# A-SHOJAEI/preference-guided-image-captioning-alignment

Hardware: NVIDIA B200
Metric: dpo_pair_tokens_per_s (higher is better)
Workload: dtype bf16

## Files before the change

### include/pgica.h

```cpp
#ifndef PGICA_H_
#define PGICA_H_

#include <stddef.h>
#include <stdint.h>

#ifdef __cplusplus
extern "C" {
#endif

#define PGICA_ABI_VERSION 1

#define PGICA_OK 0
#define PGICA_ERR_INVALID_ARGUMENT (-1)
#define PGICA_ERR_CUDA (-2)
#define PGICA_ERR_UNSUPPORTED_DEVICE (-3)
#define PGICA_ERR_WORKSPACE_TOO_SMALL (-4)

#define PGICA_MASK_NONE 0
#define PGICA_MASK_I64 1
#define PGICA_MASK_F32 2
#define PGICA_MASK_U8 3
#define PGICA_MASK_I32 4

int pgica_abi_version(void);
// ... 47 lines not shown
int pgica_lmhead_logprob_fwd(const void* hidden, const void* weight, const int64_t* labels, const void* mask,
                             int mask_kind, int64_t nseq, int64_t seqlen, int64_t d, int64_t vocab,
                             int length_normalize, float* seq_logp, float* lse, float* ztgt, int32_t* row_label,
                             float* row_weight, float* nll_sum, void* workspace, size_t workspace_bytes,
                             void* stream);
int pgica_lmhead_logprob_bwd(const void* hidden, const void* weight, const int32_t* row_label,
                             const float* row_weight, const float* lse, const float* grad_seq, int64_t nseq,
                             int64_t seqlen, int64_t d, int64_t vocab, int length_normalize, void* dhidden,
                             int dhidden_is_bf16, void* dweight, int dweight_is_bf16, void* workspace,
                             size_t workspace_bytes, void* stream);
int pgica_lmhead_logprob_bwd_progress(const void* hidden, const void* weight, const int32_t* row_label,
                                      const float* row_weight, const float* lse, const float* grad_seq, int64_t nseq,
                                      int64_t seqlen, int64_t d, int64_t vocab, int length_normalize, void* dhidden,
                                      int dhidden_is_bf16, void* dweight, uint32_t* progress, int64_t rows_per_segment,
                                      int32_t* increments_per_256_rows_host, void* workspace, size_t workspace_bytes,
                                      void* stream);

int pgica_compact_rows(const float* row_weight, int64_t rows, int32_t* index, int32_t* count, void* stream);
int pgica_gather_rows_bf16(const void* src, int src_is_bf16, const int32_t* index, int64_t n, int64_t d,
                           void* dst_bf16, const int32_t* label_in, int32_t* label_out, void* stream);
int pgica_gather_u32(const void* src, const int32_t* index, int64_t n, void* dst, void* stream);
int pgica_scatter_u32(const void* src, const int32_t* index, int64_t n, void* dst, int64_t dst_n, void* stream);
int pgica_scatter_rows(const void* src, int src_is_bf16, const int32_t* index, int64_t n, int64_t d, void* dst,
                       int dst_is_bf16, int64_t dst_rows, void* stream);
int pgica_lmhead_rows_workspace_bytes(int64_t rows, int64_t d, int64_t vocab, size_t* bytes_host);
int pgica_lmhead_rows_bwd(const void* hidden, const void* weight, const int32_t* row_label, const float* lse,
                          const float* ncoef, int64_t rows, int64_t d, int64_t vocab, void* dhidden,
                          int dhidden_is_bf16, void* dweight, int dweight_is_bf16, void* workspace,
                          size_t workspace_bytes, void* stream);

int pgica_dpo_loss_fwd(const float* pc, const float* pr, const float* rc, const float* rr, int64_t n,
                       int64_t n_global, float beta, float label_smoothing, float* loss, float* metrics, float* dpc,
                       void* stream);

int pgica_ntxent_workspace_bytes(int64_t rows_a, int64_t rows_b, int64_t dim, size_t* bytes_host);
int pgica_ntxent_fwd(const void* a, const void* b, int64_t rows_a, int64_t rows_b, int64_t dim, float inv_tau,
                     int64_t diag_offset, float* lse_row, float* diag, float* lse_col_part, void* workspace,
                     size_t workspace_bytes, void* stream);
int pgica_ntxent_fwd_bounded(const void* a, const void* b, int64_t rows_a, int64_t rows_b, int64_t dim, float inv_tau,
                             int64_t diag_offset, float* lse_row, float* diag, float* lse_col_part, void* workspace,
                             size_t workspace_bytes, void* stream);
int pgica_ntxent_bwd(const void* a, const void* b, int64_t rows_a, int64_t rows_b, int64_t dim, float inv_tau,
                     int64_t diag_offset, const float* lse_row, const float* lse_col, const float* grad_loss,
                     float grad_mult, void* da, int da_is_bf16, void* db, int db_is_bf16, void* workspace,
                     size_t workspace_bytes, void* stream);
int pgica_ntxent_bwd_bounded(const void* a, const void* b, int64_t rows_a, int64_t rows_b, int64_t dim, float inv_tau,
                             int64_t diag_offset, const float* lse_row, const float* lse_col, const float* grad_loss,
                             float grad_mult, void* da, int da_is_bf16, void* db, int db_is_bf16, void* workspace,
                             size_t workspace_bytes, void* stream);
int pgica_ntxent_loss(const float* lse_row, const float* diag, const float* lse_col_owned, int64_t n,
                      float inv_denom, float* loss, void* stream);
int pgica_lse_combine(const float* parts, int64_t nparts, int64_t n, float* out, void* stream);
int pgica_ntxent_coef(const float* grad, float mult, int64_t n, int64_t tgt_offset, int64_t tgt_limit, float* coef,
                      int32_t* tgt, void* stream);

int pgica_rownorm_fwd(const void* x, int x_is_bf16, int64_t rows, int64_t dim, float eps, void* y_bf16,
                      float* inv_norm, void* left3_bf16, void* right3_bf16, void* stream);
int pgica_rownorm_bwd(const void* x, int x_is_bf16, const float* inv_norm, const void* g, int g_is_bf16, int64_t rows,
                      int64_t dim, int64_t g_pitch, int64_t g_second, float* dx, void* stream);
int pgica_cast_f32_to_bf16(const float* x, int64_t n, void* y_bf16, void* stream);
int pgica_split3_bf16(const float* x, int64_t rows, int64_t dim, void* left3_bf16, void* right3_bf16, void* stream);

int pgica_sum_into_f32(float* dst, const void* const* srcs_host, int n_src, int64_t n, int max_ctas, void* stream);

int pgica_prep_rows(const int64_t* labels, const void* mask, int mask_kind, int64_t nseq, int64_t seqlen,
                    int64_t vocab, int32_t* row_label, float* row_weight, void* stream);
// ... 48 lines not shown
```

### preference_guided_image_captioning_alignment_b200/csrc/gemm_lse.cu

```cuda
#include "common.h"
#include "ptx.cuh"

namespace pgica {

namespace {

constexpr int kBlockM = 128;
constexpr int kBlockN = 256;
constexpr int kBlockK = 64;
constexpr int kUmmaK = 16;
constexpr int kStages = 7;
constexpr int kAccStages = 2;
constexpr uint32_t kABytes = kBlockM * kBlockK * 2;
constexpr uint32_t kBBytes = (kBlockN / 2) * kBlockK * 2;
constexpr int kMaxEpiGroups = 2;
constexpr int epi_groups(bool cols) { return cols ? 2 : 1; }
constexpr int block_threads(bool cols) { return 128 + 128 * epi_groups(cols); }
constexpr int kEpilogueWarp0 = 4;
constexpr float kLn2 = 0.6931471805599453f;

struct GemmLseParams {
  int rows, cols, k;
  int num_m_blocks, num_m_pairs, num_n_tiles, rows_pad;
  int num_parts;
// ... 233 lines not shown
        run_m = m_new;
        if ((rel >> 5) == ch && rel >= 0) {
          const int jj = rel & 31;
          float z = 0.f;
#pragma unroll
          for (int j = 0; j < 32; ++j)
            if (j == jj) z = v[j];
          run_t = z * p.scale;
        }
      }
      tc_fence_before_sync();
      mbar_arrive_cluster(&tempty_bar[acc], 0);
      if (++acc == kAccStages) {
        acc = 0;
        acc_phase ^= 1;
      }
      if (m_blk < p.num_m_blocks) {
        const size_t o = (static_cast<size_t>(n_tile) * kEpiGroups + wg) * p.rows_pad + m_blk * kBlockM + row_in_blk;
        p.part_max[o] = run_m;
        p.part_sum[o] = run_s;
        p.part_tgt[o] = run_t;
      }
    }
  }

  tc_fence_before_sync();
  __syncthreads();
  cluster_sync_all();
  if (warp == 2)
    asm volatile("tcgen05.dealloc.cta_group::2.sync.aligned.b32 %0, %1;" ::"r"(tmem_base), "r"(kAccStages * kBlockN)
                 : "memory");
}

constexpr int kMergeRows = 32, kMergeGroups = 8;
__global__ void __launch_bounds__(kMergeRows* kMergeGroups)
lse_merge_kernel(const GemmLseParams p, float* __restrict__ lse, float* __restrict__ tgt) {
  __shared__ float s_m[kMergeGroups][kMergeRows], s_s[kMergeGroups][kMergeRows], s_t[kMergeGroups][kMergeRows];
  const int r = threadIdx.x % kMergeRows, g = threadIdx.x / kMergeRows;
  const int row = blockIdx.x * kMergeRows + r;
  float m = -INFINITY, sum = 0.f, t = -INFINITY;
  if (row < p.rows) {
    for (int s = g; s < p.num_parts; s += kMergeGroups) {
      const size_t o = static_cast<size_t>(s) * p.rows_pad + row;
      const float pm = p.part_max[o], ps = p.part_sum[o];
      if (pm == -INFINITY && ps == 0.f) continue;
      const float mn = fmaxf(m, pm);
      sum = sum * exp2f(m - mn) + ps * exp2f(pm - mn);
      m = mn;
      t = fmaxf(t, p.part_tgt[o]);
    }
  }
  s_m[g][r] = m;
  s_s[g][r] = sum;
  s_t[g][r] = t;
  __syncthreads();
  if (g == 0 && row < p.rows) {
    float M = -INFINITY;
#pragma unroll
    for (int i = 0; i < kMergeGroups; ++i) M = fmaxf(M, s_m[i][r]);
    float S = 0.f, T = -INFINITY;
    bool bad = false;
#pragma unroll
    for (int i = 0; i < kMergeGroups; ++i) {
      const float mi = s_m[i][r], si = s_s[i][r];
      bad |= (si != si) || (mi != mi);
      if (mi > -INFINITY) S += si * exp2f(mi - M);
      T = fmaxf(T, s_t[i][r]);
    }
    float out = (M + log2f(S)) * kLn2;
    if (bad) out = NAN;
    lse[row] = out;
    if (tgt) tgt[row] = (T == -INFINITY) ? 0.f : T;
  }
}

__global__ void __launch_bounds__(512) col_merge_kernel(const GemmLseParams p, int groups, float* __restrict__ lse_col) {
  __shared__ float sm_m[16][33], sm_s[16][33];
  const int tx = threadIdx.x & 31, ty = threadIdx.x >> 5;
  const int j = blockIdx.x * 32 + tx;
  const size_t shift_pitch = static_cast<size_t>(p.num_n_tiles) * 8;
  const int slot = blockIdx.x;
  float M = -INFINITY, S = 0.f;
  if (j < p.cols) {
#pragma unroll 4
    for (int g = ty; g < groups; g += 16) {
      const float sh = p.col_shift[g * shift_pitch + slot];
      const float v = p.col_sum[static_cast<size_t>(g) * p.cols_pad + j];
      if (sh > -INFINITY) {
        if (sh > M) {
          S = S * exp2f(M - sh) + v;
          M = sh;
        } else {
          S += v * exp2f(sh - M);
        }
      }
    }
  }
  sm_m[ty][tx] = M;
  sm_s[ty][tx] = S;
  __syncthreads();
  if (ty == 0 && j < p.cols) {
    float Mx = -INFINITY;
#pragma unroll
    for (int t = 0; t < 16; ++t) Mx = fmaxf(Mx, sm_m[t][tx]);
    float Sx = 0.f;
#pragma unroll
// ... 13 lines not shown
  p->k = (int)k;
  p->num_m_blocks = (int)ceil_div(rows, kBlockM);
  p->num_m_pairs = (p->num_m_blocks + 1) / 2;
  p->num_n_tiles = (int)ceil_div(cols, kBlockN);
  p->rows_pad = p->num_m_blocks * kBlockM;
  const int64_t total = (int64_t)p->num_m_pairs * p->num_n_tiles;
  PGICA_REQUIRE(total < (1ll << 30), "gemm_lse: too many tiles");
  const int pairs = device_sm_count() / 2;
  *grid = 2 * (int)(total < pairs ? total : pairs);
  *ws_bytes = 3 * align_up((size_t)p->num_n_tiles * kMaxEpiGroups * p->rows_pad * sizeof(float), 256);
  return PGICA_OK;
}

size_t col_stats_bytes(const GemmLseParams& p, size_t* sum_bytes) {
  const size_t groups = static_cast<size_t>(p.rows_pad) / 32;
  const size_t cols_pad = align_up((size_t)p.cols, 32);
  *sum_bytes = align_up(groups * cols_pad * sizeof(float), 256);
  return *sum_bytes + align_up(groups * (size_t)p.num_n_tiles * 8 * sizeof(float), 256);
}

}
}

extern "C" {

int pgica_gemm_lse_workspace_bytes(int64_t rows, int64_t cols, int64_t k, size_t* bytes_host) {
  pgica::GemmLseParams p{};
  int grid = 0;
  return pgica::plan(rows, cols, k, &p, &grid, bytes_host);
}

static int gemm_lse_impl(const void* a, const void* b, int64_t rows, int64_t cols, int64_t k, float scale,
                         const int32_t* labels, int64_t diag_offset, float* lse, float* tgt, float* z_out,
                         void* workspace, size_t workspace_bytes, void* stream, float* lse_col = nullptr) {
  using namespace pgica;
  int rc = pgica_device_check();
  if (rc != PGICA_OK) return rc;
  GemmLseParams p{};
  int grid = 0;
  size_t need = 0;
  rc = plan(rows, cols, k, &p, &grid, &need);
  if (rc != PGICA_OK) return rc;
  PGICA_REQUIRE(a && b && lse, "gemm_lse: null operand");
  PGICA_REQUIRE(scale > 0.f && scale == scale, "gemm_lse: scale must be positive (got %g)", (double)scale);
  size_t col_sum_bytes = 0;
  const size_t col_bytes = lse_col ? col_stats_bytes(p, &col_sum_bytes) : 0;
  if (workspace_bytes < need + col_bytes || !workspace) {
    set_error("gemm_lse: workspace too small (%zu < %zu)", workspace_bytes, need + col_bytes);
    return PGICA_ERR_WORKSPACE_TOO_SMALL;
  }
  if (lse_col) {
    p.col_sum = reinterpret_cast<float*>(static_cast<uint8_t*>(workspace) + need);
    p.col_shift = reinterpret_cast<float*>(static_cast<uint8_t*>(workspace) + need + col_sum_bytes);
    p.cols_pad = (int)align_up((size_t)cols, 32);
  }
  const size_t seg = need / 3;
  p.part_max = reinterpret_cast<float*>(workspace);
  p.part_sum = reinterpret_cast<float*>(static_cast<uint8_t*>(workspace) + seg);
  p.part_tgt = reinterpret_cast<float*>(static_cast<uint8_t*>(workspace) + 2 * seg);
  p.num_parts = p.num_n_tiles * epi_groups(lse_col != nullptr);
  p.scale = scale;
  p.labels = labels;
  p.diag_offset = (int)diag_offset;
  p.z_out = z_out;

  CUtensorMap tm_a, tm_b;
  rc = make_tmap_bf16(&tm_a, a, rows, k, k, kBlockM);
  if (rc != PGICA_OK) return rc;
  rc = make_tmap_bf16(&tm_b, b, cols, k, k, kBlockN / 2);
  if (rc != PGICA_OK) return rc;

  cudaStream_t st = static_cast<cudaStream_t>(stream);
  auto kern = lse_col ? gemm_lse_kernel<true> : gemm_lse_kernel<false>;
  PGICA_CUDA_OK(cudaFuncSetAttribute(kern, cudaFuncAttributeMaxDynamicSharedMemorySize, (int)kSmemBytes));
  cudaLaunchConfig_t cfg{};
  cfg.gridDim = dim3((unsigned)grid);
  cfg.blockDim = dim3(lse_col ? block_threads(true) : block_threads(false));
  cfg.dynamicSmemBytes = kSmemBytes;
  cfg.stream = st;
  cudaLaunchAttribute attr[1];
  attr[0].id = cudaLaunchAttributeClusterDimension;
  attr[0].val.clusterDim.x = 2;
  attr[0].val.clusterDim.y = 1;
  attr[0].val.clusterDim.z = 1;
  cfg.attrs = attr;
  cfg.numAttrs = 1;
  PGICA_CUDA_OK(cudaLaunchKernelEx(&cfg, kern, tm_a, tm_b, p));
  count_launches(1);
  lse_merge_kernel<<<(unsigned)ceil_div(rows, kMergeRows), kMergeRows * kMergeGroups, 0, st>>>(p, lse, tgt);
  PGICA_CUDA_OK(cudaGetLastError());
  count_launches(1);
  if (lse_col) {
    col_merge_kernel<<<(unsigned)ceil_div(cols, 32), 512, 0, st>>>(p, p.rows_pad / 32, lse_col);
    PGICA_CUDA_OK(cudaGetLastError());
    count_launches(1);
  }
  return PGICA_OK;
}

int pgica_gemm_lse_rowcol_workspace_bytes(int64_t rows, int64_t cols, int64_t k, size_t* bytes_host) {
  pgica::GemmLseParams p{};
  int grid = 0;
  size_t need = 0;
  int rc = pgica::plan(rows, cols, k, &p, &grid, &need);
  if (rc != PGICA_OK) return rc;
  PGICA_REQUIRE(bytes_host, "workspace query: null result pointer");
  size_t sum_bytes = 0;
  *bytes_host = need + pgica::col_stats_bytes(p, &sum_bytes);
  return PGICA_OK;
}

int pgica_gemm_lse_rowcol(const void* a, const void* b, int64_t rows, int64_t cols, int64_t k, float scale,
                          const int32_t* labels, int64_t diag_offset, float* lse_row, float* tgt, float* lse_col,
                          void* workspace, size_t workspace_bytes, void* stream) {
  PGICA_REQUIRE(lse_col, "gemm_lse_rowcol: null column output");
  return gemm_lse_impl(a, b, rows, cols, k, scale, labels, diag_offset, lse_row, tgt, nullptr, workspace,
                       workspace_bytes, stream, lse_col);
}

int pgica_gemm_lse(const void* a, const void* b, int64_t rows, int64_t cols, int64_t k, float scale,
                   const int32_t* labels, int64_t diag_offset, float* lse, float* tgt, void* workspace,
                   size_t workspace_bytes, void* stream) {
  return gemm_lse_impl(a, b, rows, cols, k, scale, labels, diag_offset, lse, tgt, nullptr, workspace,
                       workspace_bytes, stream);
}

int pgica_similarity(const void* a, const void* b, int64_t rows, int64_t cols, int64_t k, float scale, float* sim,
                     float* lse, void* workspace, size_t workspace_bytes, void* stream) {
  PGICA_REQUIRE(sim && lse, "similarity: null output");
  return gemm_lse_impl(a, b, rows, cols, k, scale, nullptr, 0, lse, nullptr, sim, workspace, workspace_bytes, stream);
}

}
```

### preference_guided_image_captioning_alignment_b200/csrc/heads.cu

```cuda
#include "common.h"
#include "sgg_tile.cuh"

namespace pgica {
size_t sggx_workspace_bytes();
bool sggf_supported(int64_t mx, int64_t my, int64_t k);
bool sggf_single_chunk(int64_t mx, int64_t my, int64_t k);
size_t sggf_workspace_bytes();
int sggf_dispatch(const void* x, const void* y, int64_t mx, int64_t my, int64_t k, const SoftmaxGradStats& stats,
                  void* out_x, int out_x_is_bf16, void* out_y, int out_y_is_bf16, void* workspace,
                  size_t workspace_bytes, cudaStream_t st, uint32_t* progress, int64_t rows_per_segment,
                  bool shared_exponential);

namespace {
size_t backward_workspace_bytes(int64_t mx, int64_t my, int64_t k) {
  const size_t one = sggx_workspace_bytes();
  return sggf_supported(mx, my, k) && sggf_workspace_bytes() > one ? sggf_workspace_bytes() : one;
}

int backward(const void* x, const void* y, int64_t mx, int64_t my, int64_t k, float scale, const SoftmaxGradStats& st,
             void* out_x, int out_x_is_bf16, void* out_y, int out_y_is_bf16, void* ws, size_t ws_bytes, void* stream,
             bool shared_exponential) {
  if (out_x && out_y && sggf_supported(mx, my, k) && ws && ws_bytes >= sggf_workspace_bytes() &&
      (!out_y_is_bf16 || sggf_single_chunk(mx, my, k))) {
    if (shared_exponential)
      return sggf_dispatch(x, y, mx, my, k, st, out_x, out_x_is_bf16, out_y, out_y_is_bf16, ws, ws_bytes,
                           static_cast<cudaStream_t>(stream), nullptr, 0, true);
    return pgica_softmax_grad_gemm_dual(x, y, mx, my, k, scale, st.r_lse, st.r_coef, st.r_tgt, st.c_lse, st.c_coef,
                                        st.c_tgt, out_x, out_x_is_bf16, out_y, out_y_is_bf16, ws, ws_bytes, stream);
  }
  int rc;
  if (out_x) {
    rc = pgica_softmax_grad_gemm(x, y, mx, my, k, scale, st.r_lse, st.r_coef, st.r_tgt, st.c_lse, st.c_coef, st.c_tgt,
                                 out_x, out_x_is_bf16, ws, ws_bytes, stream);
    if (rc != PGICA_OK) return rc;
  }
  if (out_y) {
    const SoftmaxGradStats t = st.transposed();
    rc = pgica_softmax_grad_gemm(y, x, my, mx, k, scale, t.r_lse, t.r_coef, t.r_tgt, t.c_lse, t.c_coef, t.c_tgt, out_y,
                                 out_y_is_bf16, ws, ws_bytes, stream);
    if (rc != PGICA_OK) return rc;
  }
  return PGICA_OK;
}
}
}

using namespace pgica;

extern "C" {


int pgica_lmhead_logprob_workspace_bytes(int64_t nseq, int64_t seqlen, int64_t d, int64_t vocab, size_t* bytes_host) {
  PGICA_REQUIRE(bytes_host, "workspace query: null result pointer");
  size_t g = 0;
  int rc = pgica_gemm_lse_workspace_bytes(nseq * seqlen, vocab, d, &g);
  if (rc != PGICA_OK) return rc;
  const size_t bwd =
      align_up((size_t)(nseq * seqlen) * sizeof(float), 256) + backward_workspace_bytes(nseq * seqlen, vocab, d);
  *bytes_host = g > bwd ? g : bwd;
  return PGICA_OK;
}

int pgica_lmhead_logprob_fwd(const void* hidden, const void* weight, const int64_t* labels, const void* mask,
                             int mask_kind, int64_t nseq, int64_t seqlen, int64_t d, int64_t vocab,
                             int length_normalize, float* seq_logp, float* lse, float* ztgt, int32_t* row_label,
                             float* row_weight, float* nll_sum, void* workspace, size_t workspace_bytes,
                             void* stream) {
  PGICA_REQUIRE(hidden && weight && labels && seq_logp && lse && ztgt && row_label && row_weight,
                "lmhead_logprob_fwd: null pointer");
  int rc = pgica_prep_rows(labels, mask, mask_kind, nseq, seqlen, vocab, row_label, row_weight, stream);
  if (rc != PGICA_OK) return rc;
  rc = pgica_gemm_lse(hidden, weight, nseq * seqlen, vocab, d, 1.0f, row_label, 0, lse, ztgt, workspace,
                      workspace_bytes, stream);
  if (rc != PGICA_OK) return rc;
  return pgica_seq_reduce(lse, ztgt, row_weight, nseq, seqlen, length_normalize, seq_logp, nll_sum, stream);
}

int pgica_lmhead_rows_workspace_bytes(int64_t rows, int64_t d, int64_t vocab, size_t* bytes_host) {
  return pgica_lmhead_logprob_workspace_bytes(rows, 1, d, vocab, bytes_host);
}

int pgica_lmhead_rows_bwd(const void* hidden, const void* weight, const int32_t* row_label, const float* lse,
                          const float* ncoef, int64_t rows, int64_t d, int64_t vocab, void* dhidden,
                          int dhidden_is_bf16, void* dweight, int dweight_is_bf16, void* workspace,
                          size_t workspace_bytes, void* stream) {
  PGICA_REQUIRE(hidden && weight && row_label && lse && ncoef, "lmhead_rows_bwd: null pointer");
  PGICA_REQUIRE(dhidden || dweight, "lmhead_rows_bwd: nothing to compute");
  return backward(hidden, weight, rows, vocab, d, 1.0f, {kLog2e, lse, ncoef, row_label, nullptr, nullptr, nullptr},
                  dhidden, dhidden_is_bf16, dweight, dweight_is_bf16, workspace, workspace_bytes, stream, false);
}

int pgica_lmhead_logprob_bwd(const void* hidden, const void* weight, const int32_t* row_label,
                             const float* row_weight, const float* lse, const float* grad_seq, int64_t nseq,
                             int64_t seqlen, int64_t d, int64_t vocab, int length_normalize, void* dhidden,
                             int dhidden_is_bf16, void* dweight, int dweight_is_bf16, void* workspace,
                             size_t workspace_bytes, void* stream) {
  PGICA_REQUIRE(hidden && weight && row_label && row_weight && lse && grad_seq, "lmhead_logprob_bwd: null pointer");
  PGICA_REQUIRE(dhidden || dweight, "lmhead_logprob_bwd: nothing to compute");
  const int64_t rows = nseq * seqlen;
  if (!workspace || workspace_bytes < (size_t)rows * sizeof(float)) {
    set_error("lmhead_logprob_bwd: workspace too small (%zu < %zu)", workspace_bytes, (size_t)rows * sizeof(float));
    return PGICA_ERR_WORKSPACE_TOO_SMALL;
  }
  float* ncoef = static_cast<float*>(workspace);
  const size_t coef_bytes = align_up((size_t)rows * sizeof(float), 256);
  void* xws = workspace_bytes > coef_bytes ? static_cast<uint8_t*>(workspace) + coef_bytes : nullptr;
  const size_t xws_bytes = xws ? workspace_bytes - coef_bytes : 0;
  int rc = pgica_row_coef(grad_seq, row_weight, nseq, seqlen, length_normalize, -1.0f, ncoef, stream);
// ... 123 lines not shown
```

### preference_guided_image_captioning_alignment_b200/csrc/small.cu

```cuda
#include "common.h"
#include "ptx.cuh"

namespace pgica {
namespace {

constexpr float kLn2 = 0.6931471805599453f;

__device__ __forceinline__ float load_mask(const void* mask, int kind, size_t i) {
  switch (kind) {
    case PGICA_MASK_I64: return static_cast<float>(static_cast<const long long*>(mask)[i]);
    case PGICA_MASK_F32: return static_cast<const float*>(mask)[i];
    case PGICA_MASK_U8: return static_cast<float>(static_cast<const unsigned char*>(mask)[i]);
    case PGICA_MASK_I32: return static_cast<float>(static_cast<const int*>(mask)[i]);
    default: return 1.f;
  }
}

__global__ void prep_rows_kernel(const long long* __restrict__ labels, const void* __restrict__ mask, int mask_kind,
                                 int nseq, int T, int vocab, int* __restrict__ row_label,
                                 float* __restrict__ row_weight) {
  const size_t r = blockIdx.x * (size_t)blockDim.x + threadIdx.x;
  if (r >= (size_t)nseq * T) return;
  const int t = (int)(r % T);
  int lab = -1;
  float w = 0.f;
  if (t + 1 < T) {
    const long long y = labels[r + 1];
    w = load_mask(mask, mask_kind, r + 1);
    lab = (y >= 0 && y < vocab) ? (int)y : -1;
    if (lab < 0 && w != 0.f) w = NAN;
  }
  row_label[r] = lab;
  row_weight[r] = w;
}

__global__ void seq_reduce_kernel(const float* __restrict__ lse, const float* __restrict__ ztgt,
                                  const float* __restrict__ row_weight, int nseq, int T, int length_normalize,
                                  float* __restrict__ seq_logp, float* __restrict__ nll_sum) {
  const int b = blockIdx.x * (blockDim.x >> 5) + (threadIdx.x >> 5);
  const int lane = threadIdx.x & 31;
  if (b >= nseq) return;
  float s = 0.f, wsum = 0.f, nll = 0.f;
  for (int t = lane; t + 1 < T; t += 32) {
    const size_t r = (size_t)b * T + t;
    const float lp = ztgt[r] - lse[r];
    const float w = row_weight[r];
    s = fmaf(w, lp, s);
    wsum += w;
    nll -= lp;
  }
  s = warp_sum(s);
  wsum = warp_sum(wsum);
  nll = warp_sum(nll);
  if (lane == 0) {
    seq_logp[b] = length_normalize ? s / wsum : s;
    if (nll_sum) atomicAdd(nll_sum, nll);
  }
}

__global__ void row_coef_kernel(const float* __restrict__ grad_seq, const float* __restrict__ row_weight, int nseq,
                                int T, int length_normalize, float sign, float* __restrict__ coef) {
  const int b = blockIdx.x * (blockDim.x >> 5) + (threadIdx.x >> 5);
  const int lane = threadIdx.x & 31;
  if (b >= nseq) return;
  float wsum = 0.f;
  if (length_normalize) {
    for (int t = lane; t < T; t += 32) wsum += row_weight[(size_t)b * T + t];
    wsum = warp_sum(wsum);
  }
  const float g = grad_seq[b] * sign * (length_normalize ? 1.f / wsum : 1.f);
  for (int t = lane; t < T; t += 32) {
    const size_t r = (size_t)b * T + t;
    const float w = row_weight[r];
    coef[r] = (w == 0.f) ? 0.f : g * w;
  }
}

__global__ void dpo_loss_kernel(const float* __restrict__ pc, const float* __restrict__ pr,
                                const float* __restrict__ rc, const float* __restrict__ rr, int n, float beta,
                                float label_smoothing, float inv_n_global, float* __restrict__ loss,
                                float* __restrict__ metrics, float* __restrict__ dpc) {
  __shared__ float red[5][32];
  float acc[5] = {0.f, 0.f, 0.f, 0.f, 0.f};
  for (int i = threadIdx.x; i < n; i += blockDim.x) {
    const float pol = pc[i] - pr[i];
    const float ref = rc ? rc[i] - rr[i] : 0.f;
    const float x = beta * (pol - ref);
    const float sp_neg = fmaxf(-x, 0.f) + log1pf(expf(-fabsf(x)));
    const float sp_pos = sp_neg + x;
    const float sig_neg = 1.f / (1.f + expf(x));
// ... 8 lines not shown
    }
    dpc[i] = beta * dx * inv_n_global;
    acc[0] += l;
    acc[1] += pol - ref;
    acc[2] += (pol > ref) ? 1.f : 0.f;
    acc[3] += pc[i];
    acc[4] += pr[i];
  }
  const int warp = threadIdx.x >> 5, lane = threadIdx.x & 31;
#pragma unroll
  for (int k = 0; k < 5; ++k) {
    const float v = warp_sum(acc[k]);
    if (lane == 0) red[k][warp] = v;
  }
  __syncthreads();
  if (warp == 0) {
    const int nw = blockDim.x >> 5;
#pragma unroll
    for (int k = 0; k < 5; ++k) {
      float v = lane < nw ? red[k][lane] : 0.f;
      v = warp_sum(v);
      if (lane == 0) {
        const float m = v * inv_n_global;
        if (k == 0) *loss = m;
        metrics[k] = m;
      }
    }
  }
}

__global__ void scale_by_scalar_kernel(const float* __restrict__ a, const float* __restrict__ s, float mult, int n,
                                       float* __restrict__ out) {
  const int i = blockIdx.x * blockDim.x + threadIdx.x;
  if (i < n) out[i] = a[i] * s[0] * mult;
}

__global__ void ntxent_loss_kernel(const float* __restrict__ lse_row, const float* __restrict__ diag,
                                   const float* __restrict__ lse_col_owned, int n, float inv_denom,
                                   float* __restrict__ loss) {
  __shared__ float red[32];
  float acc = 0.f;
  for (int i = threadIdx.x; i < n; i += blockDim.x) acc += (lse_row[i] - diag[i]) + (lse_col_owned[i] - diag[i]);
  const int warp = threadIdx.x >> 5, lane = threadIdx.x & 31;
  acc = warp_sum(acc);
  if (lane == 0) red[warp] = acc;
  __syncthreads();
  if (warp == 0) {
    float v = lane < (blockDim.x >> 5) ? red[lane] : 0.f;
    v = warp_sum(v);
    if (lane == 0) *loss = 0.5f * v * inv_denom;
  }
}

__global__ void lse_combine_kernel(const float* __restrict__ parts, int nparts, int n, float* __restrict__ out) {
  const int j = blockIdx.x * blockDim.x + threadIdx.x;
  if (j >= n) return;
  float m = -INFINITY;
  for (int r = 0; r < nparts; ++r) m = fmaxf(m, parts[(size_t)r * n + j]);
  float s = 0.f;
  for (int r = 0; r < nparts; ++r) s += exp2f((parts[(size_t)r * n + j] - m) * kLog2e);
  out[j] = m + log2f(s) * kLn2;
}

__global__ void ntxent_coef_kernel(const float* __restrict__ grad, float mult, int n, int tgt_offset, int tgt_limit,
                                   float* __restrict__ coef, int* __restrict__ tgt) {
  const int i = blockIdx.x * blockDim.x + threadIdx.x;
  if (i >= n) return;
// ... 158 lines not shown
    const int lab = row_label[r];
    ztgt[r] = lab >= 0 ? ldf(z, lab) : 0.f;
  }
}

template <typename T>
__device__ __forceinline__ void stf(T* p, size_t i, float v);
template <>
__device__ __forceinline__ void stf<float>(float* p, size_t i, float v) { p[i] = v; }
template <>
__device__ __forceinline__ void stf<__nv_bfloat16>(__nv_bfloat16* p, size_t i, float v) { p[i] = __float2bfloat16(v); }

template <typename T>
__global__ void __launch_bounds__(256)
logits_grad_kernel(const T* __restrict__ logits, const int* __restrict__ row_label, const float* __restrict__ lse,
                   const float* __restrict__ coef, int vocab, T* __restrict__ dlogits) {
  const size_t r = blockIdx.x;
  const float c = coef[r];
  const T* z = logits + r * (size_t)vocab;
  T* dz = dlogits + r * (size_t)vocab;
  if (c == 0.f) {
    for (int v = threadIdx.x; v < vocab; v += blockDim.x) stf(dz, v, 0.f);
    return;
  }
  const float l2 = lse[r] * kLog2e;
  const int lab = row_label[r];
  for (int v = threadIdx.x; v < vocab; v += blockDim.x) {
    const float p = fast_exp2(ldf(z, v) * kLog2e - l2);
    stf(dz, v, c * ((v == lab ? 1.f : 0.f) - p));
  }
}

}
}

extern "C" {

using namespace pgica;

int pgica_prep_rows(const int64_t* labels, const void* mask, int mask_kind, int64_t nseq, int64_t seqlen,
                    int64_t vocab, int32_t* row_label, float* row_weight, void* stream) {
  PGICA_REQUIRE(labels && row_label && row_weight, "prep_rows: null pointer");
  PGICA_REQUIRE(nseq > 0 && seqlen > 1 && vocab > 0, "prep_rows: need nseq > 0, seqlen > 1, vocab > 0");
  PGICA_REQUIRE(mask_kind == PGICA_MASK_NONE || mask, "prep_rows: mask pointer missing for mask_kind %d", mask_kind);
  PGICA_REQUIRE(mask_kind >= PGICA_MASK_NONE && mask_kind <= PGICA_MASK_I32, "prep_rows: unknown mask_kind %d",
                mask_kind);
  const int64_t n = nseq * seqlen;
  PGICA_REQUIRE(n < (1ll << 31), "prep_rows: too many rows");
  prep_rows_kernel<<<(unsigned)ceil_div(n, 256), 256, 0, (cudaStream_t)stream>>>(
      reinterpret_cast<const long long*>(labels), mask, mask_kind, (int)nseq, (int)seqlen, (int)vocab, row_label,
      row_weight);
  PGICA_CUDA_OK(cudaGetLastError());
  count_launches(1);
  return PGICA_OK;
}

int pgica_seq_reduce(const float* lse, const float* ztgt, const float* row_weight, int64_t nseq, int64_t seqlen,
                     int length_normalize, float* seq_logp, float* nll_sum, void* stream) {
  PGICA_REQUIRE(lse && ztgt && row_weight && seq_logp, "seq_reduce: null pointer");
  PGICA_REQUIRE(nseq > 0 && seqlen > 1, "seq_reduce: bad shape");
  if (nll_sum) PGICA_CUDA_OK(cudaMemsetAsync(nll_sum, 0, sizeof(float), (cudaStream_t)stream));
  seq_reduce_kernel<<<(unsigned)ceil_div(nseq, 4), 128, 0, (cudaStream_t)stream>>>(
      lse, ztgt, row_weight, (int)nseq, (int)seqlen, length_normalize, seq_logp, nll_sum);
  PGICA_CUDA_OK(cudaGetLastError());
  count_launches(1);
  return PGICA_OK;
}

int pgica_row_coef(const float* grad_seq, const float* row_weight, int64_t nseq, int64_t seqlen, int length_normalize,
                   float sign, float* coef, void* stream) {
  PGICA_REQUIRE(grad_seq && row_weight && coef, "row_coef: null pointer");
  row_coef_kernel<<<(unsigned)ceil_div(nseq, 4), 128, 0, (cudaStream_t)stream>>>(
      grad_seq, row_weight, (int)nseq, (int)seqlen, length_normalize, sign, coef);
  PGICA_CUDA_OK(cudaGetLastError());
  count_launches(1);
  return PGICA_OK;
}

int pgica_dpo_loss_fwd(const float* pc, const float* pr, const float* rc, const float* rr, int64_t n,
                       int64_t n_global, float beta, float label_smoothing, float* loss, float* metrics, float* dpc,
                       void* stream) {
  PGICA_REQUIRE(pc && pr && loss && metrics && dpc, "dpo_loss: null pointer");
  PGICA_REQUIRE((rc == nullptr) == (rr == nullptr), "dpo_loss: reference log-probs must come as a pair");
  PGICA_REQUIRE(n > 0 && n < (1 << 24) && n_global >= n, "dpo_loss: bad pair count");
  PGICA_REQUIRE(label_smoothing >= 0.f && label_smoothing <= 1.f, "dpo_loss: label_smoothing outside [0,1]");
  dpo_loss_kernel<<<1, 256, 0, (cudaStream_t)stream>>>(pc, pr, rc, rr, (int)n, beta, label_smoothing,
                                                       1.f / (float)n_global, loss, metrics, dpc);
  PGICA_CUDA_OK(cudaGetLastError());
  count_launches(1);
  return PGICA_OK;
}

int pgica_scale_by_scalar(const float* a, const float* scalar, float mult, int64_t n, float* out, void* stream) {
  PGICA_REQUIRE(a && scalar && out && n > 0, "scale_by_scalar: bad argument");
  scale_by_scalar_kernel<<<(unsigned)ceil_div(n, 256), 256, 0, (cudaStream_t)stream>>>(a, scalar, mult, (int)n, out);
  PGICA_CUDA_OK(cudaGetLastError());
  count_launches(1);
  return PGICA_OK;
}

int pgica_ntxent_loss(const float* lse_row, const float* diag, const float* lse_col_owned, int64_t n,
                      float inv_denom, float* loss, void* stream) {
  PGICA_REQUIRE(lse_row && diag && lse_col_owned && loss && n > 0, "ntxent_loss: bad argument");
  ntxent_loss_kernel<<<1, 1024, 0, (cudaStream_t)stream>>>(lse_row, diag, lse_col_owned, (int)n, inv_denom, loss);
  PGICA_CUDA_OK(cudaGetLastError());
  count_launches(1);
  return PGICA_OK;
}

int pgica_lse_combine(const float* parts, int64_t nparts, int64_t n, float* out, void* stream) {
  PGICA_REQUIRE(parts && out && nparts > 0 && n > 0, "lse_combine: bad argument");
  lse_combine_kernel<<<(unsigned)ceil_div(n, 256), 256, 0, (cudaStream_t)stream>>>(parts, (int)nparts, (int)n, out);
  PGICA_CUDA_OK(cudaGetLastError());
  count_launches(1);
  return PGICA_OK;
}

int pgica_ntxent_coef(const float* grad, float mult, int64_t n, int64_t tgt_offset, int64_t tgt_limit, float* coef,
                      int32_t* tgt, void* stream) {
  PGICA_REQUIRE(grad && coef && tgt && n > 0, "ntxent_coef: bad argument");
  ntxent_coef_kernel<<<(unsigned)ceil_div(n, 256), 256, 0, (cudaStream_t)stream>>>(grad, mult, (int)n, (int)tgt_offset,
                                                                                  (int)tgt_limit, coef, tgt);
  PGICA_CUDA_OK(cudaGetLastError());
  count_launches(1);
  return PGICA_OK;
}

int pgica_rownorm_fwd(const void* x, int x_is_bf16, int64_t rows, int64_t dim, float eps, void* y_bf16,
// ... 120 lines not shown
```

### preference_guided_image_captioning_alignment_b200/functional.py

```python
import ctypes

import torch

from . import _lib

MASK_NONE, MASK_I64, MASK_F32, MASK_U8, MASK_I32 = 0, 1, 2, 3, 4


def _p(t):
    return None if t is None else ctypes.c_void_p(t.data_ptr())


def _stream():
    return ctypes.c_void_p(torch.cuda.current_stream().cuda_stream)


def _need_cuda(*tensors):
    for t in tensors:
        if t is not None and not t.is_cuda:
            raise _lib.PgicaError(
                "pgica ops run on a B200 only (got a %s tensor); there is no CPU fallback" % t.device.type)


def _ws(nbytes, device):
# ... 151 lines not shown
    grad_seq = grad_seq.contiguous().float()
    _lib.check(lib.pgica_lmhead_logprob_bwd(_p(hidden), _p(weight), _p(row_label), _p(row_weight), _p(lse),
                                            _p(grad_seq), nseq, T, d, V, 1 if length_normalize else 0, _p(dh),
                                            1 if dhidden_dtype == torch.bfloat16 else 0, _p(dw),
                                            1 if dweight_dtype == torch.bfloat16 else 0, _p(ws), ws.numel(),
                                            _stream()))
    return dh, dw


def dpo_loss_fwd(pc, pr, rc=None, rr=None, beta=0.1, label_smoothing=0.0, n_global=None):
    _need_cuda(pc, pr, rc, rr)
    lib = _lib.load()
    n = pc.numel()
    f32 = dict(dtype=torch.float32, device=pc.device)
    loss = torch.empty((), **f32)
    metrics = torch.empty(5, **f32)
    dpc = torch.empty(n, **f32)
    _lib.check(lib.pgica_dpo_loss_fwd(_p(pc), _p(pr), _p(rc), _p(rr), n, int(n_global or n), float(beta),
                                      float(label_smoothing), _p(loss), _p(metrics), _p(dpc), _stream()))
    return loss, metrics, dpc


def scale_by_scalar(a, scalar, mult=1.0):
    lib = _lib.load()
    out = torch.empty_like(a)
    _lib.check(lib.pgica_scale_by_scalar(_p(a), _p(scalar), float(mult), a.numel(), _p(out), _stream()))
    return out


def dpo_grad_seq(dpc, grad_loss):
    lib = _lib.load()
    n = dpc.numel()
    out = torch.empty(2 * n, dtype=torch.float32, device=dpc.device)
    g = grad_loss.reshape(1)
    _lib.check(lib.pgica_scale_by_scalar(_p(dpc), _p(g), 1.0, n, _p(out), _stream()))
    _lib.check(lib.pgica_scale_by_scalar(_p(dpc), _p(g), -1.0, n, ctypes.c_void_p(out.data_ptr() + 4 * n), _stream()))
    return out


def ntxent_fwd(a, b, inv_tau, diag_offset=0, bounded=False):
    _need_cuda(a, b)
    lib = _lib.load()
    ra, dim = a.shape
    rb = b.shape[0]
    need = ctypes.c_size_t(0)
    _lib.check(lib.pgica_ntxent_workspace_bytes(ra, rb, dim, ctypes.byref(need)))
    ws = _ws(need.value, a.device)
    f32 = dict(dtype=torch.float32, device=a.device)
    lse_row, diag, lse_col = torch.empty(ra, **f32), torch.empty(ra, **f32), torch.empty(rb, **f32)
    fn = lib.pgica_ntxent_fwd_bounded if bounded else lib.pgica_ntxent_fwd
    _lib.check(fn(_p(a), _p(b), ra, rb, dim, float(inv_tau), int(diag_offset), _p(lse_row), _p(diag), _p(lse_col), _p(ws),
                  need.value, _stream()))
    return lse_row, diag, lse_col


def ntxent_loss(lse_row, diag, lse_col_owned, inv_denom):
    lib = _lib.load()
    loss = torch.empty((), dtype=torch.float32, device=lse_row.device)
    _lib.check(lib.pgica_ntxent_loss(_p(lse_row), _p(diag), _p(lse_col_owned), lse_row.numel(), float(inv_denom),
                                     _p(loss), _stream()))
    return loss


def lse_combine(parts):
    lib = _lib.load()
    parts = parts.contiguous()
    out = torch.empty(parts.shape[1], dtype=torch.float32, device=parts.device)
    _lib.check(lib.pgica_lse_combine(_p(parts), parts.shape[0], parts.shape[1], _p(out), _stream()))
    return out
# ... 425 lines not shown
```

Measured before the change: 1.414 million.

## Fuse sequence log-prob reduction into LSE merge via per-sequence tickets

Folds the per-sequence log-prob reduction into the LSE merge kernel. A per-sequence atomic ticket lets the last merge block that finishes a sequence compute its weighted sum, and ticket and NLL zeroing move into the prep_rows kernel. This removes the separate seq_reduce launch and the memset. The merge loop now batches partial loads (16 ahead) to raise memory-level parallelism, and the two DPO grad scale launches become a single 2-D launch. The cost is extra workspace for tickets, threadfence/atomic overhead, and more register pressure in the merge kernel.

```diff
diff --git a/include/pgica.h b/include/pgica.h
--- a/include/pgica.h
+++ b/include/pgica.h
@@ -103,6 +103,7 @@
 int pgica_dpo_loss_fwd(const float* pc, const float* pr, const float* rc, const float* rr, int64_t n,
                        int64_t n_global, float beta, float label_smoothing, float* loss, float* metrics, float* dpc,
                        void* stream);
+int pgica_dpo_grad_seq(const float* dpc, const float* grad_loss, int64_t n, float* out, void* stream);
 
 int pgica_ntxent_workspace_bytes(int64_t rows_a, int64_t rows_b, int64_t dim, size_t* bytes_host);
 int pgica_ntxent_fwd(const void* a, const void* b, int64_t rows_a, int64_t rows_b, int64_t dim, float inv_tau,
diff --git a/preference_guided_image_captioning_alignment_b200/csrc/gemm_lse.cu b/preference_guided_image_captioning_alignment_b200/csrc/gemm_lse.cu
--- a/preference_guided_image_captioning_alignment_b200/csrc/gemm_lse.cu
+++ b/preference_guided_image_captioning_alignment_b200/csrc/gemm_lse.cu
@@ -289,22 +289,69 @@
                  : "memory");
 }
 
-constexpr int kMergeRows = 32, kMergeGroups = 8;
+struct SeqSums {
+  const float* row_weight;
+  int T;
+  int length_normalize;
+  float* seq_logp;
+  float* nll_sum;
+  unsigned* ticket;
+};
+
+__device__ __forceinline__ void seq_sum_warp(const float* __restrict__ lse, const float* __restrict__ ztgt,
+                                             const float* __restrict__ row_weight, int b, int T, int length_normalize,
+                                             float* __restrict__ seq_logp, float* __restrict__ nll_sum) {
+  const int lane = threadIdx.x & 31;
+  float s = 0.f, wsum = 0.f, nll = 0.f;
+#pragma unroll 4
+  for (int t = lane; t + 1 < T; t += 32) {
+    const size_t r = (size_t)b * T + t;
+    const float lp = __ldcg(ztgt + r) - __ldcg(lse + r);
+    const float w = row_weight[r];
+    s = fmaf(w, lp, s);
+    wsum += w;
+    nll -= lp;
+  }
+  s = warp_sum(s);
+  wsum = warp_sum(wsum);
+  nll = warp_sum(nll);
+  if (lane == 0) {
+    seq_logp[b] = length_normalize ? s / wsum : s;
+    if (nll_sum) atomicAdd(nll_sum, nll);
+  }
+}
+
+constexpr int kMergeRows = 32, kMergeGroups = 8, kMergeAhead = 16;
 __global__ void __launch_bounds__(kMergeRows* kMergeGroups)
-lse_merge_kernel(const GemmLseParams p, float* __restrict__ lse, float* __restrict__ tgt) {
+lse_merge_kernel(const GemmLseParams p, float* __restrict__ lse, float* __restrict__ tgt, const SeqSums q) {
   __shared__ float s_m[kMergeGroups][kMergeRows], s_s[kMergeGroups][kMergeRows], s_t[kMergeGroups][kMergeRows];
   const int r = threadIdx.x % kMergeRows, g = threadIdx.x / kMergeRows;
   const int row = blockIdx.x * kMergeRows + r;
   float m = -INFINITY, sum = 0.f, t = -INFINITY;
   if (row < p.rows) {
-    for (int s = g; s < p.num_parts; s += kMergeGroups) {
-      const size_t o = static_cast<size_t>(s) * p.rows_pad + row;
-      const float pm = p.part_max[o], ps = p.part_sum[o];
-      if (pm == -INFINITY && ps == 0.f) continue;
-      const float mn = fmaxf(m, pm);
-      sum = sum * exp2f(m - mn) + ps * exp2f(pm - mn);
-      m = mn;
-      t = fmaxf(t, p.part_tgt[o]);
+    for (int s0 = g; s0 < p.num_parts; s0 += kMergeGroups * kMergeAhead) {
+      float pm[kMergeAhead], ps[kMergeAhead], pt[kMergeAhead];
+#pragma unroll
+      for (int i = 0; i < kMergeAhead; ++i) {
+        const int s = s0 + i * kMergeGroups;
+        pm[i] = -INFINITY;
+        ps[i] = 0.f;
+        pt[i] = -INFINITY;
+        if (s < p.num_parts) {
+          const size_t o = static_cast<size_t>(s) * p.rows_pad + row;
+          pm[i] = p.part_max[o];
+          ps[i] = p.part_sum[o];
+          pt[i] = p.part_tgt[o];
+        }
+      }
+#pragma unroll
+      for (int i = 0; i < kMergeAhead; ++i) {
+        if (pm[i] == -INFINITY && ps[i] == 0.f) continue;
+        const float mn = fmaxf(m, pm[i]);
+        sum = sum * exp2f(m - mn) + ps[i] * exp2f(pm[i] - mn);
+        m = mn;
+        t = fmaxf(t, pt[i]);
+      }
     }
   }
   s_m[g][r] = m;
@@ -329,6 +376,33 @@
     lse[row] = out;
     if (tgt) tgt[row] = (T == -INFINITY) ? 0.f : T;
   }
+  if (q.seq_logp == nullptr) return;
+
+  __shared__ int s_done[kMergeRows], s_ndone;
+  if (threadIdx.x == 0) s_ndone = 0;
+  __syncthreads();
+  const int r0 = blockIdx.x * kMergeRows, r1 = min(r0 + kMergeRows, p.rows) - 1;
+  const int b0 = r0 / q.T, nb = r1 / q.T - b0 + 1;
+  if ((int)threadIdx.x < nb) {
+    const int b = b0 + threadIdx.x;
+    const int blocks = ((b + 1) * q.T - 1) / kMergeRows - b * q.T / kMergeRows + 1;
+    __threadfence();
+    if (atomicAdd(&q.ticket[b], 1u) == (unsigned)(blocks - 1)) s_done[atomicAdd(&s_ndone, 1)] = b;
+  }
+  __syncthreads();
+  const int ndone = s_ndone;
+  if (ndone == 0) return;
+  __threadfence();
+  for (int i = threadIdx.x >> 5; i < ndone; i += blockDim.x >> 5)
+    seq_sum_warp(lse, tgt, q.row_weight, s_done[i], q.T, q.length_normalize, q.seq_logp, q.nll_sum);
+}
+
+__global__ void seq_reduce_kernel(const float* __restrict__ lse, const float* __restrict__ ztgt,
+                                  const float* __restrict__ row_weight, int nseq, int T, int length_normalize,
+                                  float* __restrict__ seq_logp, float* __restrict__ nll_sum) {
+  const int b = blockIdx.x * (blockDim.x >> 5) + (threadIdx.x >> 5);
+  if (b >= nseq) return;
+  seq_sum_warp(lse, ztgt, row_weight, b, T, length_normalize, seq_logp, nll_sum);
 }
 
 __global__ void __launch_bounds__(512) col_merge_kernel(const GemmLseParams p, int groups, float* __restrict__ lse_col) {
@@ -408,7 +482,8 @@
 
 static int gemm_lse_impl(const void* a, const void* b, int64_t rows, int64_t cols, int64_t k, float scale,
                          const int32_t* labels, int64_t diag_offset, float* lse, float* tgt, float* z_out,
-                         void* workspace, size_t workspace_bytes, void* stream, float* lse_col = nullptr) {
+                         void* workspace, size_t workspace_bytes, void* stream, float* lse_col = nullptr,
+                         const pgica::SeqSums& seq = {}) {
   using namespace pgica;
   int rc = pgica_device_check();
   if (rc != PGICA_OK) return rc;
@@ -463,7 +538,7 @@
   cfg.numAttrs = 1;
   PGICA_CUDA_OK(cudaLaunchKernelEx(&cfg, kern, tm_a, tm_b, p));
   count_launches(1);
-  lse_merge_kernel<<<(unsigned)ceil_div(rows, kMergeRows), kMergeRows * kMergeGroups, 0, st>>>(p, lse, tgt);
+  lse_merge_kernel<<<(unsigned)ceil_div(rows, kMergeRows), kMergeRows * kMergeGroups, 0, st>>>(p, lse, tgt, seq);
   PGICA_CUDA_OK(cudaGetLastError());
   count_launches(1);
   if (lse_col) {
@@ -507,4 +582,32 @@
   return gemm_lse_impl(a, b, rows, cols, k, scale, nullptr, 0, lse, nullptr, sim, workspace, workspace_bytes, stream);
 }
 
-}
+int pgica_seq_reduce(const float* lse, const float* ztgt, const float* row_weight, int64_t nseq, int64_t seqlen,
+                     int length_normalize, float* seq_logp, float* nll_sum, void* stream) {
+  using namespace pgica;
+  PGICA_REQUIRE(lse && ztgt && row_weight && seq_logp, "seq_reduce: null pointer");
+  PGICA_REQUIRE(nseq > 0 && seqlen > 1, "seq_reduce: bad shape");
+  if (nll_sum) PGICA_CUDA_OK(cudaMemsetAsync(nll_sum, 0, sizeof(float), (cudaStream_t)stream));
+  seq_reduce_kernel<<<(unsigned)ceil_div(nseq, 4), 128, 0, (cudaStream_t)stream>>>(
+      lse, ztgt, row_weight, (int)nseq, (int)seqlen, length_normalize, seq_logp, nll_sum);
+  PGICA_CUDA_OK(cudaGetLastError());
+  count_launches(1);
+  return PGICA_OK;
+}
+
+}
+
+namespace pgica {
+
+int gemm_lse_seq(const void* hidden, const void* weight, int64_t nseq, int64_t seqlen, int64_t d, int64_t vocab,
+                 const int32_t* row_label, const float* row_weight, int length_normalize, float* lse, float* ztgt,
+                 float* seq_logp, float* nll_sum, uint32_t* ticket, void* workspace, size_t workspace_bytes,
+                 void* stream) {
+  PGICA_REQUIRE(ztgt && row_weight && seq_logp && ticket, "gemm_lse_seq: null pointer");
+  PGICA_REQUIRE(seqlen > 1, "gemm_lse_seq: seqlen must be > 1");
+  const SeqSums seq{row_weight, (int)seqlen, length_normalize, seq_logp, nll_sum, ticket};
+  return gemm_lse_impl(hidden, weight, nseq * seqlen, vocab, d, 1.0f, row_label, 0, lse, ztgt, nullptr, workspace,
+                       workspace_bytes, stream, nullptr, seq);
+}
+
+}
diff --git a/preference_guided_image_captioning_alignment_b200/csrc/heads.cu b/preference_guided_image_captioning_alignment_b200/csrc/heads.cu
--- a/preference_guided_image_captioning_alignment_b200/csrc/heads.cu
+++ b/preference_guided_image_captioning_alignment_b200/csrc/heads.cu
@@ -10,6 +10,12 @@
                   void* out_x, int out_x_is_bf16, void* out_y, int out_y_is_bf16, void* workspace,
                   size_t workspace_bytes, cudaStream_t st, uint32_t* progress, int64_t rows_per_segment,
                   bool shared_exponential);
+int prep_rows(const int64_t* labels, const void* mask, int mask_kind, int64_t nseq, int64_t seqlen, int64_t vocab,
+              int32_t* row_label, float* row_weight, uint32_t* ticket, float* nll_sum, void* stream);
+int gemm_lse_seq(const void* hidden, const void* weight, int64_t nseq, int64_t seqlen, int64_t d, int64_t vocab,
+                 const int32_t* row_label, const float* row_weight, int length_normalize, float* lse, float* ztgt,
+                 float* seq_logp, float* nll_sum, uint32_t* ticket, void* workspace, size_t workspace_bytes,
+                 void* stream);
 
 namespace {
 size_t backward_workspace_bytes(int64_t mx, int64_t my, int64_t k) {
@@ -55,9 +61,10 @@
   size_t g = 0;
   int rc = pgica_gemm_lse_workspace_bytes(nseq * seqlen, vocab, d, &g);
   if (rc != PGICA_OK) return rc;
+  const size_t fwd = g + align_up((size_t)nseq * sizeof(uint32_t), 256);
   const size_t bwd =
       align_up((size_t)(nseq * seqlen) * sizeof(float), 256) + backward_workspace_bytes(nseq * seqlen, vocab, d);
-  *bytes_host = g > bwd ? g : bwd;
+  *bytes_host = fwd > bwd ? fwd : bwd;
   return PGICA_OK;
 }
 
@@ -68,12 +75,19 @@
                              void* stream) {
   PGICA_REQUIRE(hidden && weight && labels && seq_logp && lse && ztgt && row_label && row_weight,
                 "lmhead_logprob_fwd: null pointer");
-  int rc = pgica_prep_rows(labels, mask, mask_kind, nseq, seqlen, vocab, row_label, row_weight, stream);
-  if (rc != PGICA_OK) return rc;
-  rc = pgica_gemm_lse(hidden, weight, nseq * seqlen, vocab, d, 1.0f, row_label, 0, lse, ztgt, workspace,
-                      workspace_bytes, stream);
-  if (rc != PGICA_OK) return rc;
-  return pgica_seq_reduce(lse, ztgt, row_weight, nseq, seqlen, length_normalize, seq_logp, nll_sum, stream);
+  size_t g = 0;
+  int rc = pgica_gemm_lse_workspace_bytes(nseq * seqlen, vocab, d, &g);
+  if (rc != PGICA_OK) return rc;
+  if (!workspace || workspace_bytes < g + (size_t)nseq * sizeof(uint32_t)) {
+    set_error("lmhead_logprob_fwd: workspace too small (%zu < %zu)", workspace_bytes,
+              g + (size_t)nseq * sizeof(uint32_t));
+    return PGICA_ERR_WORKSPACE_TOO_SMALL;
+  }
+  uint32_t* ticket = reinterpret_cast<uint32_t*>(static_cast<uint8_t*>(workspace) + g);
+  rc = prep_rows(labels, mask, mask_kind, nseq, seqlen, vocab, row_label, row_weight, ticket, nll_sum, stream);
+  if (rc != PGICA_OK) return rc;
+  return gemm_lse_seq(hidden, weight, nseq, seqlen, d, vocab, row_label, row_weight, length_normalize, lse, ztgt,
+                      seq_logp, nll_sum, ticket, workspace, g, stream);
 }
 
 int pgica_lmhead_rows_workspace_bytes(int64_t rows, int64_t d, int64_t vocab, size_t* bytes_host) {
diff --git a/preference_guided_image_captioning_alignment_b200/csrc/small.cu b/preference_guided_image_captioning_alignment_b200/csrc/small.cu
--- a/preference_guided_image_captioning_alignment_b200/csrc/small.cu
+++ b/preference_guided_image_captioning_alignment_b200/csrc/small.cu
@@ -18,9 +18,12 @@
 
 __global__ void prep_rows_kernel(const long long* __restrict__ labels, const void* __restrict__ mask, int mask_kind,
                                  int nseq, int T, int vocab, int* __restrict__ row_label,
-                                 float* __restrict__ row_weight) {
+                                 float* __restrict__ row_weight, unsigned* __restrict__ ticket,
+                                 float* __restrict__ nll_sum) {
   const size_t r = blockIdx.x * (size_t)blockDim.x + threadIdx.x;
   if (r >= (size_t)nseq * T) return;
+  if (ticket && r < (size_t)nseq) ticket[r] = 0u;
+  if (nll_sum && r == 0) *nll_sum = 0.f;
   const int t = (int)(r % T);
   int lab = -1;
   float w = 0.f;
@@ -32,30 +35,6 @@
   }
   row_label[r] = lab;
   row_weight[r] = w;
-}
-
-__global__ void seq_reduce_kernel(const float* __restrict__ lse, const float* __restrict__ ztgt,
-                                  const float* __restrict__ row_weight, int nseq, int T, int length_normalize,
-                                  float* __restrict__ seq_logp, float* __restrict__ nll_sum) {
-  const int b = blockIdx.x * (blockDim.x >> 5) + (threadIdx.x >> 5);
-  const int lane = threadIdx.x & 31;
-  if (b >= nseq) return;
-  float s = 0.f, wsum = 0.f, nll = 0.f;
-  for (int t = lane; t + 1 < T; t += 32) {
-    const size_t r = (size_t)b * T + t;
-    const float lp = ztgt[r] - lse[r];
-    const float w = row_weight[r];
-    s = fmaf(w, lp, s);
-    wsum += w;
-    nll -= lp;
-  }
-  s = warp_sum(s);
-  wsum = warp_sum(wsum);
-  nll = warp_sum(nll);
-  if (lane == 0) {
-    seq_logp[b] = length_normalize ? s / wsum : s;
-    if (nll_sum) atomicAdd(nll_sum, nll);
-  }
 }
 
 __global__ void row_coef_kernel(const float* __restrict__ grad_seq, const float* __restrict__ row_weight, int nseq,
@@ -130,7 +109,7 @@
 __global__ void scale_by_scalar_kernel(const float* __restrict__ a, const float* __restrict__ s, float mult, int n,
                                        float* __restrict__ out) {
   const int i = blockIdx.x * blockDim.x + threadIdx.x;
-  if (i < n) out[i] = a[i] * s[0] * mult;
+  if (i < n) out[(size_t)blockIdx.y * n + i] = a[i] * s[0] * (blockIdx.y ? -mult : mult);
 }
 
 __global__ void ntxent_loss_kernel(const float* __restrict__ lse_row, const float* __restrict__ diag,
@@ -355,14 +334,9 @@
 }
 
 }
-}
-
-extern "C" {
-
-using namespace pgica;
-
-int pgica_prep_rows(const int64_t* labels, const void* mask, int mask_kind, int64_t nseq, int64_t seqlen,
-                    int64_t vocab, int32_t* row_label, float* row_weight, void* stream) {
+
+int prep_rows(const int64_t* labels, const void* mask, int mask_kind, int64_t nseq, int64_t seqlen, int64_t vocab,
+              int32_t* row_label, float* row_weight, uint32_t* ticket, float* nll_sum, void* stream) {
   PGICA_REQUIRE(labels && row_label && row_weight, "prep_rows: null pointer");
   PGICA_REQUIRE(nseq > 0 && seqlen > 1 && vocab > 0, "prep_rows: need nseq > 0, seqlen > 1, vocab > 0");
   PGICA_REQUIRE(mask_kind == PGICA_MASK_NONE || mask, "prep_rows: mask pointer missing for mask_kind %d", mask_kind);
@@ -372,22 +346,21 @@
   PGICA_REQUIRE(n < (1ll << 31), "prep_rows: too many rows");
   prep_rows_kernel<<<(unsigned)ceil_div(n, 256), 256, 0, (cudaStream_t)stream>>>(
       reinterpret_cast<const long long*>(labels), mask, mask_kind, (int)nseq, (int)seqlen, (int)vocab, row_label,
-      row_weight);
-  PGICA_CUDA_OK(cudaGetLastError());
-  count_launches(1);
-  return PGICA_OK;
-}
-
-int pgica_seq_reduce(const float* lse, const float* ztgt, const float* row_weight, int64_t nseq, int64_t seqlen,
-                     int length_normalize, float* seq_logp, float* nll_sum, void* stream) {
-  PGICA_REQUIRE(lse && ztgt && row_weight && seq_logp, "seq_reduce: null pointer");
-  PGICA_REQUIRE(nseq > 0 && seqlen > 1, "seq_reduce: bad shape");
-  if (nll_sum) PGICA_CUDA_OK(cudaMemsetAsync(nll_sum, 0, sizeof(float), (cudaStream_t)stream));
-  seq_reduce_kernel<<<(unsigned)ceil_div(nseq, 4), 128, 0, (cudaStream_t)stream>>>(
-      lse, ztgt, row_weight, (int)nseq, (int)seqlen, length_normalize, seq_logp, nll_sum);
-  PGICA_CUDA_OK(cudaGetLastError());
-  count_launches(1);
-  return PGICA_OK;
+      row_weight, ticket, nll_sum);
+  PGICA_CUDA_OK(cudaGetLastError());
+  count_launches(1);
+  return PGICA_OK;
+}
+
+}
+
+extern "C" {
+
+using namespace pgica;
+
+int pgica_prep_rows(const int64_t* labels, const void* mask, int mask_kind, int64_t nseq, int64_t seqlen,
+                    int64_t vocab, int32_t* row_label, float* row_weight, void* stream) {
+  return prep_rows(labels, mask, mask_kind, nseq, seqlen, vocab, row_label, row_weight, nullptr, nullptr, stream);
 }
 
 int pgica_row_coef(const float* grad_seq, const float* row_weight, int64_t nseq, int64_t seqlen, int length_normalize,
@@ -417,6 +390,15 @@
 int pgica_scale_by_scalar(const float* a, const float* scalar, float mult, int64_t n, float* out, void* stream) {
   PGICA_REQUIRE(a && scalar && out && n > 0, "scale_by_scalar: bad argument");
   scale_by_scalar_kernel<<<(unsigned)ceil_div(n, 256), 256, 0, (cudaStream_t)stream>>>(a, scalar, mult, (int)n, out);
+  PGICA_CUDA_OK(cudaGetLastError());
+  count_launches(1);
+  return PGICA_OK;
+}
+
+int pgica_dpo_grad_seq(const float* dpc, const float* grad_loss, int64_t n, float* out, void* stream) {
+  PGICA_REQUIRE(dpc && grad_loss && out && n > 0 && n < (1ll << 30), "dpo_grad_seq: bad argument");
+  scale_by_scalar_kernel<<<dim3((unsigned)ceil_div(n, 256), 2), 256, 0, (cudaStream_t)stream>>>(dpc, grad_loss, 1.0f,
+                                                                                                 (int)n, out);
   PGICA_CUDA_OK(cudaGetLastError());
   count_launches(1);
   return PGICA_OK;
diff --git a/preference_guided_image_captioning_alignment_b200/functional.py b/preference_guided_image_captioning_alignment_b200/functional.py
--- a/preference_guided_image_captioning_alignment_b200/functional.py
+++ b/preference_guided_image_captioning_alignment_b200/functional.py
@@ -207,9 +207,7 @@
     lib = _lib.load()
     n = dpc.numel()
     out = torch.empty(2 * n, dtype=torch.float32, device=dpc.device)
-    g = grad_loss.reshape(1)
-    _lib.check(lib.pgica_scale_by_scalar(_p(dpc), _p(g), 1.0, n, _p(out), _stream()))
-    _lib.check(lib.pgica_scale_by_scalar(_p(dpc), _p(g), -1.0, n, ctypes.c_void_p(out.data_ptr() + 4 * n), _stream()))
+    _lib.check(lib.pgica_dpo_grad_seq(_p(dpc), _p(grad_loss.reshape(1)), n, _p(out), _stream()))
     return out
 
 
```

Result: no change. 1.421 million, median of 6 (+0.5%).
